# facebookresearch/iris

Measured on AMD Instinct MI355X. Metric: bake_shading throughput (shading samples/s: secondary rays traced and shaded), higher is better.
Workload: dtype f32; 1 GPU; bake_shading train-view sequence (15 views evenly spaced among 32 cameras on a circle, one view per step), 1920x1080, SPP=128 per lobe, lobes=[0, 1, 2, 3, 4, 5, 6] (0=diffuse,1-6=specular), synthetic room seed=1 1000990 triangles, SLF H=256, Philox uniforms; pixels_per_view=2073600

## Files before the change

iris_amd/csrc/iris_bake.h:

```cpp
#pragma once
#include "iris_tile.h"

namespace iris {

struct BakeArgs {
    SceneDev sc; EmitDev em; SlfDev slf;
    const float* pos; const float* nrm; const float* wo;
    const float* u2; const int32_t* pix_id;
    int64_t P; int spp; uint64_t seed; uint32_t stream_id; float rough;
    float* out0; float* out1; int64_t* tri_next;
    int64_t* src_next;
    unsigned long long* stats;
    uint32_t* stack_ovf;
    float4* scratch;
    unsigned int* tile_counter;
    int tile_px;
};

#ifndef IRIS_TILE_RAYS
#define IRIS_TILE_RAYS 5120
#endif
constexpr int kTileRays = IRIS_TILE_RAYS;

__device__ __forceinline__ void reduce_geometry(int spp, int& lpp, int& ppw, int& rounds) {
    if (spp >= 64) { lpp = 64; ppw = 1; rounds = (spp + 63) >> 6; }
    else if ((spp & (spp - 1)) == 0) { lpp = spp; ppw = 64 / spp; rounds = 1; }
    else { lpp = 64; ppw = 1; rounds = 1; }
}

struct RayOut { float r0, g0, b0, r1, g1, b1; };

template <bool SPEC>
__device__ __forceinline__ void sample_dir(const BakeArgs& a, float u0, float u1, f3 n, f3 w, f3 t, f3 b, f3& wi, float& g0, float& g1) {
    g0 = 1.f; g1 = 0.f;
    if (SPEC) {
        wi = specular_sampler(u0, u1, a.rough, w, n, t, b);
        SpecW sw = specular_weights(wi, w, n, a.rough, false);
        g0 = sw.g0; g1 = sw.g1;
    } else {
        wi = diffuse_sampler(u0, u1, n, t, b);
    }
}
template <bool SPEC>
__device__ __forceinline__ void sample_lobe(const BakeArgs& a, int64_t p, int s, f3 n, f3 w, f3 t, f3 b, uint64_t base, f3& wi, float& g0, float& g1) {
    float u0, u1;
    if (a.u2) { const float* up = a.u2 + (p * a.spp + s) * 2; u0 = up[0]; u1 = up[1]; }
    else {
        uint32_t s_lo = (uint32_t)a.seed, s_hi = (uint32_t)(a.seed >> 32);
        asm volatile("" : "+s"(s_lo), "+s"(s_hi));
        philox_u2(((uint64_t)s_hi << 32) | s_lo, base + (uint64_t)s, a.stream_id, u0, u1);
    }
    sample_dir<SPEC>(a, u0, u1, n, w, t, b, wi, g0, g1);
}

template <bool SPEC, bool COUNT, int LAYOUT, int LDS_DEPTH = kStackLds, bool GLOBAL_OVF = false>
__device__ __forceinline__ RayOut trace_shade(const BakeArgs& a, int64_t p, int s, f3 x, f3 wi, float g0, float g1, uint32_t* lds_stack,
                                              TraceStats* ts, uint32_t& n_rays, uint32_t* ovf = nullptr) {
    f3 o = mk3(x.x + kRayEps * wi.x, x.y + kRayEps * wi.y, x.z + kRayEps * wi.z);
    const uint32_t steps0 = COUNT ? ts->nodes + ts->tris : 0;
    Hit h = trace_bvh4<LAYOUT, COUNT, LDS_DEPTH, GLOBAL_OVF>(a.sc, o, wi, lds_stack, ts, ovf);
    if (COUNT) {
        n_rays++;
        uint32_t mine = ts->nodes + ts->tris - steps0, mx = mine;
        for (int m = 1; m < 64; m <<= 1) mx = max(mx, (uint32_t)__shfl_xor((int)mx, m));
        if (first_active_lane()) ts->max_steps64 += (unsigned long long)mx * 64ull;
    }
    f3 pn = mk3(0.f, 0.f, 0.f);
    int64_t tri = -1;
    if (h.slot >= 0) {
        f3 p0, p1, p2;
        hit_vertices(a.sc, h, p0, p1, p2);
        pn = hit_position(h, p0, p1, p2);
        tri = h.id;
    }
    if (a.tri_next) a.tri_next[p * a.spp + s] = tri;
    float epdf; bool vn; int src;
    f3 Le = eval_emitter1(a.em, a.slf, pn, tri, true, 1.0f, 0.0f, epdf, vn, src);
    if (a.src_next) a.src_next[p * a.spp + s] = src;
    RayOut r;
    if (SPEC) { r.r0 = Le.x * g0; r.g0 = Le.y * g0; r.b0 = Le.z * g0; r.r1 = Le.x * g1; r.g1 = Le.y * g1; r.b1 = Le.z * g1; }
    else { r.r0 = Le.x; r.g0 = Le.y; r.b0 = Le.z; r.r1 = r.g1 = r.b1 = 0.f; }
    return r;
}

template <bool SPEC, bool COUNT, int LAYOUT, int LDS_DEPTH = kStackLds, bool GLOBAL_OVF = false>
__device__ __forceinline__ RayOut shade_sample(const BakeArgs& a, int64_t p, int s, f3 x, f3 n, f3 w, f3 t, f3 b, uint64_t base,
                                               uint32_t* lds_stack, TraceStats* ts, uint32_t& n_rays, uint32_t* ovf = nullptr) {
    f3 wi; float g0, g1;
    sample_lobe<SPEC>(a, p, s, n, w, t, b, base, wi, g0, g1);
    return trace_shade<SPEC, COUNT, LAYOUT, LDS_DEPTH, GLOBAL_OVF>(a, p, s, x, wi, g0, g1, lds_stack, ts, n_rays, ovf);
}

template <bool COUNT>
__device__ __forceinline__ void flush_stats(const BakeArgs& a, const TraceStats& ts, uint32_t n_rays) {
    if (COUNT) {
        uint32_t v[8] = {n_rays, ts.nodes, ts.tris, ts.node_iters, ts.leaf_iters, ts.sp_gt8, ts.sp_gt12, ts.sp_gt16};
        for (int k = 0; k < 8; ++k) {
            uint32_t x = v[k];
            for (int m = 1; m < 64; m <<= 1) x += __shfl_xor(x, m);
            if ((threadIdx.x & 63) == 0) atomicAdd(a.stats + k, (unsigned long long)x);
        }
        uint32_t w[2] = {ts.drain_nodes, ts.drain_node_iters};
        for (int k = 0; k < 2; ++k) {
            uint32_t x = w[k];
            for (int m = 1; m < 64; m <<= 1) x += __shfl_xor(x, m);
            if ((threadIdx.x & 63) == 0) atomicAdd(a.stats + 9 + k, (unsigned long long)x);
        }
        uint32_t tp[4] = {ts.top21, ts.top85, ts.top341, ts.top1365};
        for (int k = 0; k < 4; ++k) {
            uint32_t x = tp[k];
            for (int m = 1; m < 64; m <<= 1) x += __shfl_xor(x, m);
            if ((threadIdx.x & 63) == 0) atomicAdd(a.stats + 11 + k, (unsigned long long)x);
        }
        uint32_t sh[5] = {ts.shared_iters, ts.shared_lanes, ts.shared_all_iters, ts.slow_push_iters, ts.shared_path_iters};
        for (int k = 0; k < 5; ++k) {
            uint32_t x = sh[k];
            for (int m = 1; m < 64; m <<= 1) x += __shfl_xor(x, m);
            if ((threadIdx.x & 63) == 0) atomicAdd(a.stats + 15 + k, (unsigned long long)x);
        }
        unsigned long long y = ts.max_steps64;
        for (int m = 1; m < 64; m <<= 1) y += __shfl_xor(y, m);
        if ((threadIdx.x & 63) == 0) atomicAdd(a.stats + 8, y);
    }
}

template <bool SPEC, bool COUNT, int LAYOUT>
__global__ __launch_bounds__(kBlock) void bake_kernel(BakeArgs a) {
    __shared__ uint32_t s_stack[kStackLds * kBlock];
    const int lane = threadIdx.x & 63;
    const int spp = a.spp;
    int lpp, ppw, rounds;
    reduce_geometry(spp, lpp, ppw, rounds);
    const int sub = lane / lpp, sl = lane - sub * lpp;
    const int64_t n_groups = (a.P + ppw - 1) / ppw;
    const int64_t wave0 = ((int64_t)blockIdx.x * kBlock + threadIdx.x) >> 6;
    const int64_t n_waves = ((int64_t)gridDim.x * kBlock) >> 6;
    const float inv_spp = 1.0f / (float)spp;
    TraceStats ts;
    uint32_t n_rays = 0;

    for (int64_t g = wave0; g < n_groups; g += n_waves) {
        const int64_t p = g * ppw + sub;
        const bool pvalid = p < a.P;
        f3 x = mk3(0.f, 0.f, 0.f), n = mk3(0.f, 0.f, 1.f), w = mk3(0.f, 0.f, 1.f), t, b;
        uint64_t base = 0;
        if (pvalid) {
            x = ld3(a.pos + p * 3); n = ld3(a.nrm + p * 3);
            if (SPEC) w = ld3(a.wo + p * 3);
            base = (uint64_t)(a.pix_id ? (int64_t)a.pix_id[p] : p) * (uint64_t)spp;
        }
        normal_space(n, t, b);
        float a0x = 0.f, a0y = 0.f, a0z = 0.f, a1x = 0.f, a1y = 0.f, a1z = 0.f;
        for (int r = 0; r < rounds; ++r) {
            const int s = r * 64 + sl;
            if (pvalid && s < spp) {
                RayOut o = shade_sample<SPEC, COUNT, LAYOUT>(a, p, s, x, n, w, t, b, base, s_stack + threadIdx.x, &ts, n_rays);
                a0x += o.r0; a0y += o.g0; a0z += o.b0;
                if (SPEC) { a1x += o.r1; a1y += o.g1; a1z += o.b1; }
            }
        }
        for (int m = 1; m < lpp; m <<= 1) {
            a0x += __shfl_xor(a0x, m); a0y += __shfl_xor(a0y, m); a0z += __shfl_xor(a0z, m);
            if (SPEC) { a1x += __shfl_xor(a1x, m); a1y += __shfl_xor(a1y, m); a1z += __shfl_xor(a1z, m); }
        }
        if (pvalid && sl == 0) {
            st3(a.out0 + p * 3, mk3(a0x * inv_spp, a0y * inv_spp, a0z * inv_spp));
            if (SPEC) st3(a.out1 + p * 3, mk3(a1x * inv_spp, a1y * inv_spp, a1z * inv_spp));
        }
    }
    flush_stats<COUNT>(a, ts, n_rays);
}

#ifndef IRIS_TILE_WAVES
#define IRIS_TILE_WAVES 7
#endif
#ifndef IRIS_TILE_STACK
#define IRIS_TILE_STACK 12
#endif

template <bool SPEC, bool COUNT, int LAYOUT, int TILE_STACK>
__device__ __forceinline__ void tile_body(const BakeArgs& a, int64_t p0, int np, float4* res, uint16_t* s_sorted, uint32_t* s_stack, int* s_chunk,
                                          uint32_t* ovf, TraceStats& ts, uint32_t& n_rays) {
    const int tid = threadIdx.x, lane = tid & 63, wave = tid >> 6;
    const int spp = a.spp;
    float2* res_g = reinterpret_cast<float2*>(res + kTileRays);
    int lpp, ppw, rounds;
    reduce_geometry(spp, lpp, ppw, rounds);
    const int sub = lane / lpp, sl = lane - sub * lpp;
    const float inv_spp = 1.0f / (float)spp;
    const int nr = np * spp;
    const bool resolve = !a.em.emit_ord && !a.tri_next;

    const uint32_t spp_m = spp > 1 ? (uint32_t)(0x100000000ull / (uint64_t)(uint32_t)spp) + 1u : 0u;
    auto div_spp = [&](int r) -> int { return spp > 1 ? (int)__umulhi((uint32_t)r, spp_m) : r; };

    constexpr int kFrameOff = (kTileRays + 2 * 256 * 4) / 4, kFramePx = (TILE_STACK * kBlock - kFrameOff) / 6;
    float* s_frames = reinterpret_cast<float*>(s_stack) + kFrameOff;
    const bool frames = np <= kFramePx;
    if (frames) {
        for (int pl = tid; pl < np; pl += kBlock) {
            f3 t, b;
            normal_space(ld3(a.nrm + (p0 + pl) * 3), t, b);
            float* f = s_frames + pl * 6;
            f[0] = t.x; f[1] = t.y; f[2] = t.z; f[3] = b.x; f[4] = b.y; f[5] = b.z;
        }
        __syncthreads();
    }

    tile_sort_trace<LAYOUT, COUNT, kTileRays, TILE_STACK, true>(
        a.sc, nr, s_sorted, s_stack, s_chunk, ovf, ts,
        [&](int r) -> uint32_t {
            const int pl = div_spp(r), s = r - pl * spp;
            const int64_t p = p0 + pl;
            const f3 n = ld3(a.nrm + p * 3), w = SPEC ? ld3(a.wo + p * 3) : mk3(0.f, 0.f, 1.f);
            const uint64_t base = (uint64_t)(a.pix_id ? (int64_t)a.pix_id[p] : p) * (uint64_t)spp;
            f3 t, b;
            if (frames) { const float* f = s_frames + pl * 6; t = mk3(f[0], f[1], f[2]); b = mk3(f[3], f[4], f[5]); }
            else normal_space(n, t, b);
            f3 wi; float g0, g1;
            sample_lobe<SPEC>(a, p, s, n, w, t, b, base, wi, g0, g1);
            res[r] = make_float4(wi.x, wi.y, wi.z, 0.f);
            if (SPEC) res_g[r] = make_float2(g1, g0);
            return dir_bin(wi);
        },
        [&](int r, f3& o, f3& d) {
            const int64_t p = p0 + div_spp(r);
            o = ld3(a.pos + p * 3);
            const float4 qa = res[r];
            d = mk3(qa.x, qa.y, qa.z);
        },
        [&](f3& o, f3& d) { o = mk3(o.x + kRayEps * d.x, o.y + kRayEps * d.y, o.z + kRayEps * d.z); },
        [&](int r, const Hit& h) {
            if (resolve) {
                float4 q = make_float4(0.f, 0.f, 0.f, __int_as_float(-2));
                if (h.slot >= 0) {
                    const float4* tr = a.sc.tris + (int64_t)h.slot * 4;
                    const float4 tx = tr[0], ty = tr[1], tz = tr[2];
                    const float ow = tr[3].x;
                    const f3 pn = hit_position(h, mk3(tx.x, ty.x, tz.x), mk3(tx.y, ty.y, tz.y), mk3(tx.z, ty.z, tz.z));
                    q = make_float4(pn.x, pn.y, pn.z, ow);
                }
                res[r] = q;
            } else
            res[r] = make_float4(h.u, h.v, __int_as_float(h.slot), 0.f);
            if (COUNT) n_rays++; }
        );

    const int n_groups = (np + ppw - 1) / ppw;
    IRIS_PHASE_BEGIN();
    for (int g = wave; g < n_groups; g += kBlock / 64) {
        const int pl = g * ppw + sub;
        const bool pvalid = pl < np;
        float a0x = 0.f, a0y = 0.f, a0z = 0.f, a1x = 0.f, a1y = 0.f, a1z = 0.f;
        if (resolve) {
            for (int rr = 0; rr < rounds; rr += 2) {
                const int s0 = rr * 64 + sl, s1 = s0 + 64;
                const bool ok0 = pvalid && s0 < spp, ok1 = pvalid && rr + 1 < rounds && s1 < spp;
                float4 q0 = make_float4(0.f, 0.f, 0.f, __int_as_float(-2)), q1 = q0;
                float2 w0 = make_float2(0.f, 0.f), w1 = w0;
                if (ok0) { q0 = res[pl * spp + s0]; if (SPEC) w0 = res_g[pl * spp + s0]; }
                if (ok1) { q1 = res[pl * spp + s1]; if (SPEC) w1 = res_g[pl * spp + s1]; }
                const int o0 = __float_as_int(q0.w), o1 = __float_as_int(q1.w);
                int j0 = -1, j1 = -1;
                if (o0 == -1) j0 = slf_index(a.slf, mk3(q0.x, q0.y, q0.z));
                if (o1 == -1) j1 = slf_index(a.slf, mk3(q1.x, q1.y, q1.z));
                float4 r0 = make_float4(0.f, 0.f, 0.f, 0.f), r1 = r0;
                if (o0 >= 0 || j0 >= 0) r0 = *(o0 >= 0 ? a.em.radiance + o0 : a.slf.radiance + j0);
                if (o1 >= 0 || j1 >= 0) r1 = *(o1 >= 0 ? a.em.radiance + o1 : a.slf.radiance + j1);
                if (ok0) {
                    const float z = o0 >= 0 ? -0.f : 0.f;
                    const f3 Le = mk3(z + r0.x, z + r0.y, z + r0.z);
                    if (a.src_next) a.src_next[(p0 + pl) * spp + s0] = o0 >= 0 ? -2 - o0 : j0;
                    if (SPEC) { a0x += Le.x * w0.y; a0y += Le.y * w0.y; a0z += Le.z * w0.y; a1x += Le.x * w0.x; a1y += Le.y * w0.x; a1z += Le.z * w0.x; }
                    else { a0x += Le.x; a0y += Le.y; a0z += Le.z; }
                }
                if (ok1) {
                    const float z = o1 >= 0 ? -0.f : 0.f;
                    const f3 Le = mk3(z + r1.x, z + r1.y, z + r1.z);
                    if (a.src_next) a.src_next[(p0 + pl) * spp + s1] = o1 >= 0 ? -2 - o1 : j1;
                    if (SPEC) { a0x += Le.x * w1.y; a0y += Le.y * w1.y; a0z += Le.z * w1.y; a1x += Le.x * w1.x; a1y += Le.y * w1.x; a1z += Le.z * w1.x; }
                    else { a0x += Le.x; a0y += Le.y; a0z += Le.z; }
                }
            }
        } else
        for (int rr = 0; rr < rounds; ++rr) {
            const int s = rr * 64 + sl;
            if (pvalid && s < spp) {
                const float4 qa = res[pl * spp + s];
                Hit h; h.u = qa.x; h.v = qa.y; h.slot = __float_as_int(qa.z); h.t = 0.f; h.id = 0;
                f3 pn = mk3(0.f, 0.f, 0.f);
                int64_t tri = -1;
                int ord_rec = -1;
                if (h.slot >= 0) {
                    const float4* tr = a.sc.tris + (int64_t)h.slot * 4;
                    const float4 tx = tr[0], ty = tr[1], tz = tr[2];
                    if (!a.em.emit_ord) ord_rec = __float_as_int(tr[3].x);
                    pn = hit_position(h, mk3(tx.x, ty.x, tz.x), mk3(tx.y, ty.y, tz.y), mk3(tx.z, ty.z, tz.z));
                    tri = __float_as_int(tx.w);
                }
                if (a.tri_next) a.tri_next[(p0 + pl) * spp + s] = tri;
                float epdf; bool vn; int src;
                const f3 Le = eval_emitter1(a.em, a.slf, pn, tri, true, 1.0f, 0.0f, epdf, vn, src, ord_rec);
                if (a.src_next) a.src_next[(p0 + pl) * spp + s] = src;
                if (SPEC) {
                    const float2 qb = res_g[pl * spp + s];
                    a0x += Le.x * qb.y; a0y += Le.y * qb.y; a0z += Le.z * qb.y;
                    a1x += Le.x * qb.x; a1y += Le.y * qb.x; a1z += Le.z * qb.x;
                } else { a0x += Le.x; a0y += Le.y; a0z += Le.z; }
            }
        }
        for (int m = 1; m < lpp; m <<= 1) {
            a0x += __shfl_xor(a0x, m); a0y += __shfl_xor(a0y, m); a0z += __shfl_xor(a0z, m);
            if (SPEC) { a1x += __shfl_xor(a1x, m); a1y += __shfl_xor(a1y, m); a1z += __shfl_xor(a1z, m); }
        }
        if (pvalid && sl == 0) {
            const int64_t p = p0 + pl;
            st3(a.out0 + p * 3, mk3(a0x * inv_spp, a0y * inv_spp, a0z * inv_spp));
            if (SPEC) st3(a.out1 + p * 3, mk3(a1x * inv_spp, a1y * inv_spp, a1z * inv_spp));
        }
    }
    IRIS_PHASE_MARK(3);
}

constexpr int kTileChunk = 64;
__device__ __forceinline__ long long claim_tile(unsigned int* counters, long long n_tiles) {
    constexpr int kChunk = kTileChunk;
    const long long n_chunks = (n_tiles + kChunk - 1) / kChunk;
    for (int k = 0; k < 8; ++k) {
        const int x = ((int)blockIdx.x + k) & 7;
        const long long per = (n_chunks + 7 - x) / 8;
        for (;;) {
            const unsigned int c = atomicAdd(counters + x, 1u);
            const long long ch = (long long)(c / kChunk);
            if (ch >= per) break;
            const long long t = (ch * 8 + x) * kChunk + (c % kChunk);
            if (t < n_tiles) return t;
        }
    }
    return n_tiles;
}

template <bool SPEC, bool COUNT, int LAYOUT>
__global__ __launch_bounds__(kBlock, COUNT ? 4 : IRIS_TILE_WAVES) void bake_tile_kernel(BakeArgs a) {
    constexpr int kTileStack = IRIS_TILE_STACK;
    __shared__ uint16_t s_sorted[kTileRays];
    __shared__ uint32_t s_stack[kTileStack * kBlock];
    __shared__ int s_tile, s_chunk;
    static_assert(kTileStack * kBlock * 4 >= kTileRays + 2 * 256 * 4, "stack region too small to alias the sort keys");
    const int tid = threadIdx.x;
    constexpr int NC = SPEC ? 2 : 1;
    float4* res = a.scratch + (size_t)blockIdx.x * kTileRays * NC;
    uint32_t* ovf = a.stack_ovf + (size_t)blockIdx.x * (kStackCapacity - kTileStack) * kBlock;
    const int64_t n_tiles = (a.P + a.tile_px - 1) / a.tile_px;
    TraceStats ts;
    uint32_t n_rays = 0;
    for (;;) {
        __syncthreads();
        if (tid == 0) { s_tile = (int)claim_tile(a.tile_counter, n_tiles); s_chunk = 0; }
        (s_stack + kTileRays / 4)[tid] = 0;
        __syncthreads();
        const int64_t tile = s_tile;
        if (tile >= n_tiles) break;
        const int64_t p0 = (int64_t)tile * a.tile_px;
        tile_body<SPEC, COUNT, LAYOUT, kTileStack>(a, p0, (int)min((int64_t)a.tile_px, a.P - p0), res, s_sorted, s_stack, &s_chunk, ovf, ts, n_rays);
    }
    flush_stats<COUNT>(a, ts, n_rays);
}

constexpr int kMaxLobes = 8;
struct ViewLobe { float rough; int spp; uint32_t stream_id; int spec; int tile_px; int tiles_per_span; float* out0; float* out1; };
struct ViewArgs {
    BakeArgs base;
    int n_lobes;
    int span_px;
    long long n_tiles;
    ViewLobe lobe[kMaxLobes];
};

template <int LAYOUT>
__global__ __launch_bounds__(kBlock, IRIS_TILE_WAVES) void bake_view_kernel(ViewArgs v) {
    constexpr int kTileStack = IRIS_TILE_STACK;
    __shared__ uint16_t s_sorted[kTileRays];
    __shared__ uint32_t s_stack[kTileStack * kBlock];
    __shared__ int s_tile, s_chunk;
    static_assert(kTileStack * kBlock * 4 >= kTileRays + 2 * 256 * 4, "stack region too small to alias the sort keys");
    const int tid = threadIdx.x;
    float4* res = v.base.scratch + (size_t)blockIdx.x * kTileRays * 2;
    uint32_t* ovf = v.base.stack_ovf + (size_t)blockIdx.x * (kStackCapacity - kTileStack) * kBlock;
    for (;;) {
        __syncthreads();
        if (tid == 0) { s_tile = (int)claim_tile(v.base.tile_counter, v.n_tiles); s_chunk = 0; }
        (s_stack + kTileRays / 4)[tid] = 0;
        __syncthreads();
        const long long vt = s_tile;
        if (vt >= v.n_tiles) break;
        const long long g = vt / kTileChunk, q = g >> 3;
        const int j = (int)(vt % kTileChunk), l = (int)(q % v.n_lobes);
        const int64_t span0 = ((q / v.n_lobes) * 8 + (g & 7)) * (int64_t)v.span_px;
        const int64_t p0 = span0 + (int64_t)j * v.lobe[l].tile_px;
        if (j >= v.lobe[l].tiles_per_span || p0 >= v.base.P) continue;
        const int np = (int)min((int64_t)v.lobe[l].tile_px, min(v.base.P, span0 + v.span_px) - p0);
        BakeArgs a = v.base;
        a.spp = v.lobe[l].spp; a.rough = v.lobe[l].rough; a.stream_id = v.lobe[l].stream_id; a.tile_px = v.lobe[l].tile_px;
        a.out0 = v.lobe[l].out0; a.out1 = v.lobe[l].out1; a.u2 = nullptr; a.tri_next = nullptr; a.src_next = nullptr;
        TraceStats ts; uint32_t n_rays = 0;
        if (v.lobe[l].spec) tile_body<true, false, LAYOUT, kTileStack>(a, p0, np, res, s_sorted, s_stack, &s_chunk, ovf, ts, n_rays);
        else tile_body<false, false, LAYOUT, kTileStack>(a, p0, np, res, s_sorted, s_stack, &s_chunk, ovf, ts, n_rays);
    }
}

}
```

iris_amd/csrc/iris_tile.h:

```cpp
#pragma once
#include "iris_trace.h"

namespace iris {

#ifndef IRIS_PRIO_A
#define IRIS_PRIO_A 0
#endif
#ifndef IRIS_PRIO_C
#define IRIS_PRIO_C 3
#endif
#ifndef IRIS_PRIO_D
#define IRIS_PRIO_D 0
#endif

__device__ __forceinline__ uint32_t dir_bin(f3 d) {
    const float ax = fabsf(d.x), ay = fabsf(d.y), az = fabsf(d.z);
    const float inv = __builtin_amdgcn_rcpf(ax + ay + az + 1e-30f);
    const float a = ax * inv, b = ay * inv;
    const float v = b * __builtin_amdgcn_rcpf(1.f - a + 1e-30f);
    const int iu = min(7, (int)(a * 8.f)), iv0 = min(3, (int)(v * 4.f));
    const int iv = (iu & 1) ? 3 - iv0 : iv0;
    const uint32_t oct = (d.x < 0.f ? 1u : 0u) | (d.y < 0.f ? 2u : 0u) | (d.z < 0.f ? 4u : 0u);
    return (oct << 5) | ((uint32_t)iu << 2) | (uint32_t)iv;
}

#ifdef IRIS_PHASE_TIMING
__device__ unsigned long long g_phase_cycles[8];
#define IRIS_PHASE_BEGIN() unsigned long long t_phase_ = clock64()
#define IRIS_PHASE_MARK(k) do { if (threadIdx.x == 0) { const unsigned long long t_ = clock64(); atomicAdd(&g_phase_cycles[k], t_ - t_phase_); t_phase_ = t_; } } while (0)
#else
#define IRIS_PHASE_BEGIN()
#define IRIS_PHASE_MARK(k)
#endif

template <int LAYOUT, bool COUNT, int CAP, int TILE_STACK, bool GLOBAL_OVF, class PhaseA, class FetchRay, class Prepare, class Retire>
__device__ __forceinline__ void tile_sort_trace(const SceneDev& sc, int nr, uint16_t* s_sorted, uint32_t* s_stack, int* s_chunk, uint32_t* ovf,
                                                TraceStats& ts, PhaseA phase_a, FetchRay fetch_ray, Prepare prepare, Retire retire) {
    static_assert(TILE_STACK * kBlock * 4 >= CAP + 2 * 256 * 4, "stack region too small to alias the sort keys");
    uint8_t* s_keys = reinterpret_cast<uint8_t*>(s_stack);
    uint32_t* s_hist = s_stack + CAP / 4;
    uint32_t* s_cur = s_hist + 256;
    const int tid = threadIdx.x, lane = tid & 63, wave = tid >> 6;
    IRIS_PHASE_BEGIN();
    __builtin_amdgcn_s_setprio(IRIS_PRIO_A);
    for (int r = tid; r < nr; r += kBlock) {
        const uint32_t key = phase_a(r);
        s_keys[r] = (uint8_t)key;
        atomicAdd(&s_hist[key], 1u);
    }
    __syncthreads();
    IRIS_PHASE_MARK(0);
    if (wave == 0) {
        uint32_t c0 = s_hist[lane * 4], c1 = s_hist[lane * 4 + 1], c2 = s_hist[lane * 4 + 2], c3 = s_hist[lane * 4 + 3];
        uint32_t tot = c0 + c1 + c2 + c3, inc = tot;
        for (int m = 1; m < 64; m <<= 1) { uint32_t v = __shfl_up(inc, m); if (lane >= m) inc += v; }
        uint32_t ex = inc - tot;
        s_cur[lane * 4] = ex; s_cur[lane * 4 + 1] = ex + c0; s_cur[lane * 4 + 2] = ex + c0 + c1; s_cur[lane * 4 + 3] = ex + c0 + c1 + c2;
    }
    __syncthreads();
    for (int r = tid; r < nr; r += kBlock) {
        const uint32_t pos = atomicAdd(&s_cur[s_keys[r]], 1u);
        s_sorted[pos] = (uint16_t)r;
    }
    __syncthreads();
    IRIS_PHASE_MARK(1);
    {
        int my_r = 0;
        auto fetch = [&](f3& o, f3& d) -> bool {
            const unsigned long long m = __ballot(1);
            int base = 0;
            if (lane == __ffsll((long long)m) - 1) base = atomicAdd(s_chunk, __popcll(m));
            base = __builtin_amdgcn_readfirstlane(base);
            const int i = base + (int)__builtin_amdgcn_mbcnt_hi((uint32_t)(m >> 32), __builtin_amdgcn_mbcnt_lo((uint32_t)m, 0u));
            if (i >= nr) return false;
            my_r = s_sorted[i];
            fetch_ray(my_r, o, d);
            return true;
        };
        auto ret = [&](const Hit& h) { retire(my_r, h); };
        __builtin_amdgcn_s_setprio(IRIS_PRIO_C);
        uint32_t tid_c = threadIdx.x;
        asm volatile("" : "+v"(tid_c));
        SceneDev sc_c = sc;
        asm volatile("" : "+s"(sc_c.nodes), "+s"(sc_c.tris), "+s"(sc_c.oct_stride));
        trace_stream<LAYOUT, COUNT, TILE_STACK, GLOBAL_OVF>(sc_c, s_stack + tid_c, tid_c, ovf, &ts, fetch, prepare, ret);
        __builtin_amdgcn_s_setprio(IRIS_PRIO_D);
        IRIS_PHASE_MARK(4);
    }
    __syncthreads();
    IRIS_PHASE_MARK(2);
}

}
```

Before: 9229 Mrays/s.

## Outline sampling and shading phases into noinline functions reading kernel args directly

Splits the per-tile body into separate noinline functions for sample generation/binning (phase A) and shading/accumulation (phase D). Each reloads its arguments from the kernel-argument segment, with wave-uniform parameters and global address-space pointers, and the traversal loop stays inlined. The aim is to stop register pressure from the sampling and shading code from inflating the traversal's register allocation, and to merge the spec and diffuse paths so only one traversal instance is compiled per kernel. The trade-off is call overhead, possible spills at call boundaries, and reliance on the implicit-argument layout of the kernel arguments.

```diff
diff --git a/iris_amd/csrc/iris_bake.h b/iris_amd/csrc/iris_bake.h
--- a/iris_amd/csrc/iris_bake.h
+++ b/iris_amd/csrc/iris_bake.h
@@ -178,22 +178,67 @@
 #define IRIS_TILE_STACK 12
 #endif
 
-template <bool SPEC, bool COUNT, int LAYOUT, int TILE_STACK>
-__device__ __forceinline__ void tile_body(const BakeArgs& a, int64_t p0, int np, float4* res, uint16_t* s_sorted, uint32_t* s_stack, int* s_chunk,
-                                          uint32_t* ovf, TraceStats& ts, uint32_t& n_rays) {
-    const int tid = threadIdx.x, lane = tid & 63, wave = tid >> 6;
+typedef __attribute__((address_space(4))) const char cst_char;
+template <class ARGS> __device__ __forceinline__ cst_char* kernel_args() { return (cst_char*)__builtin_amdgcn_implicitarg_ptr() - ((sizeof(ARGS) + 7) & ~(size_t)7); }
+template <class T> __device__ __forceinline__ T* as_global(T* p) { return (T*)(__attribute__((address_space(1))) T*)p; }
+__device__ __forceinline__ void globalize(BakeArgs& a) {
+    a.sc.tris = as_global(a.sc.tris); a.em.emit_ord = as_global(a.em.emit_ord); a.em.radiance = as_global(a.em.radiance);
+    a.slf.inds = as_global(a.slf.inds); a.slf.radiance = as_global(a.slf.radiance);
+    a.nrm = as_global(a.nrm); a.wo = as_global(a.wo); a.u2 = as_global(a.u2); a.pix_id = as_global(a.pix_id);
+    a.out0 = as_global(a.out0); a.out1 = as_global(a.out1); a.tri_next = as_global(a.tri_next); a.src_next = as_global(a.src_next); a.scratch = as_global(a.scratch);
+}
+struct ViewLobe { float rough; int spp; uint32_t stream_id; int spec; int tile_px; int tiles_per_span; float* out0; float* out1; };
+__device__ __forceinline__ void set_lobe(BakeArgs& a, const ViewLobe& L) {
+    a.spp = L.spp; a.rough = L.rough; a.stream_id = L.stream_id; a.tile_px = L.tile_px;
+    a.out0 = L.out0; a.out1 = L.out1; a.u2 = nullptr; a.tri_next = nullptr; a.src_next = nullptr;
+}
+constexpr int kMaxLobes = 8;
+struct ViewArgs {
+    BakeArgs base;
+    int n_lobes;
+    int span_px;
+    long long n_tiles;
+    ViewLobe lobe[kMaxLobes];
+};
+struct TileLaunch {
+    typedef BakeArgs Args;
+    template <bool SPEC> static constexpr int kSlab = SPEC ? 2 : 1;
+    __device__ static __forceinline__ BakeArgs args(cst_char* k, int) {
+        BakeArgs a;
+        __builtin_memcpy(&a, k, sizeof(BakeArgs));
+        globalize(a);
+        return a;
+    }
+};
+struct ViewLaunch {
+    typedef ViewArgs Args;
+    template <bool SPEC> static constexpr int kSlab = 2;
+    __device__ static __forceinline__ BakeArgs args(cst_char* k, int l) {
+        BakeArgs a; ViewLobe L;
+        __builtin_memcpy(&a, k + offsetof(ViewArgs, base), sizeof(BakeArgs));
+        __builtin_memcpy(&L, k + offsetof(ViewArgs, lobe) + (size_t)l * sizeof(ViewLobe), sizeof(ViewLobe));
+        set_lobe(a, L);
+        globalize(a);
+        return a;
+    }
+};
+#define IRIS_TILE_PHASE __device__ __noinline__
+__device__ __forceinline__ int64_t uniform64(int64_t x) {
+    return (int64_t)(((uint64_t)(uint32_t)__builtin_amdgcn_readfirstlane((int)((uint64_t)x >> 32)) << 32) | (uint32_t)__builtin_amdgcn_readfirstlane((int)x));
+}
+
+
+template <bool SPEC, int TILE_STACK, class LAUNCH>
+IRIS_TILE_PHASE void tile_phase_a(int l, int64_t p0, int np, lds_u32* lds) {
+    l = __builtin_amdgcn_readfirstlane(l); np = __builtin_amdgcn_readfirstlane(np); p0 = uniform64(p0);
+    const BakeArgs a = LAUNCH::args(kernel_args<typename LAUNCH::Args>(), l);
+    uint32_t* s_stack = (uint32_t*)lds;
+    float4* res = a.scratch + (size_t)blockIdx.x * kTileRays * LAUNCH::template kSlab<SPEC>;
+    float2* res_g = reinterpret_cast<float2*>(res + kTileRays);
+    const int tid = threadIdx.x;
     const int spp = a.spp;
-    float2* res_g = reinterpret_cast<float2*>(res + kTileRays);
-    int lpp, ppw, rounds;
-    reduce_geometry(spp, lpp, ppw, rounds);
-    const int sub = lane / lpp, sl = lane - sub * lpp;
-    const float inv_spp = 1.0f / (float)spp;
-    const int nr = np * spp;
-    const bool resolve = !a.em.emit_ord && !a.tri_next;
-
     const uint32_t spp_m = spp > 1 ? (uint32_t)(0x100000000ull / (uint64_t)(uint32_t)spp) + 1u : 0u;
     auto div_spp = [&](int r) -> int { return spp > 1 ? (int)__umulhi((uint32_t)r, spp_m) : r; };
-
     constexpr int kFrameOff = (kTileRays + 2 * 256 * 4) / 4, kFramePx = (TILE_STACK * kBlock - kFrameOff) / 6;
     float* s_frames = reinterpret_cast<float*>(s_stack) + kFrameOff;
     const bool frames = np <= kFramePx;
@@ -207,8 +252,7 @@
         __syncthreads();
     }
 
-    tile_sort_trace<LAYOUT, COUNT, kTileRays, TILE_STACK, true>(
-        a.sc, nr, s_sorted, s_stack, s_chunk, ovf, ts,
+    tile_bin<kTileRays>(np * spp, s_stack,
         [&](int r) -> uint32_t {
             const int pl = div_spp(r), s = r - pl * spp;
             const int64_t p = p0 + pl;
@@ -222,30 +266,22 @@
             res[r] = make_float4(wi.x, wi.y, wi.z, 0.f);
             if (SPEC) res_g[r] = make_float2(g1, g0);
             return dir_bin(wi);
-        },
-        [&](int r, f3& o, f3& d) {
-            const int64_t p = p0 + div_spp(r);
-            o = ld3(a.pos + p * 3);
-            const float4 qa = res[r];
-            d = mk3(qa.x, qa.y, qa.z);
-        },
-        [&](f3& o, f3& d) { o = mk3(o.x + kRayEps * d.x, o.y + kRayEps * d.y, o.z + kRayEps * d.z); },
-        [&](int r, const Hit& h) {
-            if (resolve) {
-                float4 q = make_float4(0.f, 0.f, 0.f, __int_as_float(-2));
-                if (h.slot >= 0) {
-                    const float4* tr = a.sc.tris + (int64_t)h.slot * 4;
-                    const float4 tx = tr[0], ty = tr[1], tz = tr[2];
-                    const float ow = tr[3].x;
-                    const f3 pn = hit_position(h, mk3(tx.x, ty.x, tz.x), mk3(tx.y, ty.y, tz.y), mk3(tx.z, ty.z, tz.z));
-                    q = make_float4(pn.x, pn.y, pn.z, ow);
-                }
-                res[r] = q;
-            } else
-            res[r] = make_float4(h.u, h.v, __int_as_float(h.slot), 0.f);
-            if (COUNT) n_rays++; }
-        );
-
+        });
+}
+
+template <bool SPEC, class LAUNCH>
+IRIS_TILE_PHASE void tile_phase_d(int l, int64_t p0, int np) {
+    l = __builtin_amdgcn_readfirstlane(l); np = __builtin_amdgcn_readfirstlane(np); p0 = uniform64(p0);
+    const BakeArgs a = LAUNCH::args(kernel_args<typename LAUNCH::Args>(), l);
+    float4* res = a.scratch + (size_t)blockIdx.x * kTileRays * LAUNCH::template kSlab<SPEC>;
+    float2* res_g = reinterpret_cast<float2*>(res + kTileRays);
+    const int tid = threadIdx.x, lane = tid & 63, wave = tid >> 6;
+    const int spp = a.spp;
+    int lpp, ppw, rounds;
+    reduce_geometry(spp, lpp, ppw, rounds);
+    const int sub = lane / lpp, sl = lane - sub * lpp;
+    const float inv_spp = 1.0f / (float)spp;
+    const bool resolve = !a.em.emit_ord && !a.tri_next;
     const int n_groups = (np + ppw - 1) / ppw;
     IRIS_PHASE_BEGIN();
     for (int g = wave; g < n_groups; g += kBlock / 64) {
@@ -322,6 +358,58 @@
     IRIS_PHASE_MARK(3);
 }
 
+template <bool SPEC, int TILE_STACK> struct TileLobe {
+    __device__ __forceinline__ void phase_a(int64_t p0, int np, uint32_t* s_stack) const { tile_phase_a<SPEC, TILE_STACK, TileLaunch>(0, p0, np, (lds_u32*)s_stack); }
+    __device__ __forceinline__ void phase_d(int64_t p0, int np) const { tile_phase_d<SPEC, TileLaunch>(0, p0, np); }
+};
+template <int TILE_STACK> struct ViewTileLobe {
+    int l; bool spec;
+    __device__ __forceinline__ void phase_a(int64_t p0, int np, uint32_t* s_stack) const {
+        if (spec) tile_phase_a<true, TILE_STACK, ViewLaunch>(l, p0, np, (lds_u32*)s_stack); else tile_phase_a<false, TILE_STACK, ViewLaunch>(l, p0, np, (lds_u32*)s_stack);
+    }
+    __device__ __forceinline__ void phase_d(int64_t p0, int np) const {
+        if (spec) tile_phase_d<true, ViewLaunch>(l, p0, np); else tile_phase_d<false, ViewLaunch>(l, p0, np);
+    }
+};
+
+template <bool COUNT, int LAYOUT, int TILE_STACK, class LOBE>
+__device__ __forceinline__ void tile_body(const BakeArgs& a, LOBE lobe, int64_t p0, int np, float4* res, uint16_t* s_sorted, uint32_t* s_stack, int* s_chunk,
+                                          uint32_t* ovf, TraceStats& ts, uint32_t& n_rays) {
+    const int spp = a.spp;
+    const int nr = np * spp;
+    const bool resolve = !a.em.emit_ord && !a.tri_next;
+    const uint32_t spp_m = spp > 1 ? (uint32_t)(0x100000000ull / (uint64_t)(uint32_t)spp) + 1u : 0u;
+    auto div_spp = [&](int r) -> int { return spp > 1 ? (int)__umulhi((uint32_t)r, spp_m) : r; };
+
+    lobe.phase_a(p0, np, s_stack);
+    tile_trace_sorted<LAYOUT, COUNT, kTileRays, TILE_STACK, true>(
+        a.sc, nr, s_sorted, s_stack, s_chunk, ovf, ts,
+        [&](int r, f3& o, f3& d) {
+            const int64_t p = p0 + div_spp(r);
+            o = ld3(a.pos + p * 3);
+            const float4 qa = res[r];
+            d = mk3(qa.x, qa.y, qa.z);
+        },
+        [&](f3& o, f3& d) { o = mk3(o.x + kRayEps * d.x, o.y + kRayEps * d.y, o.z + kRayEps * d.z); },
+        [&](int r, const Hit& h) {
+            if (resolve) {
+                float4 q = make_float4(0.f, 0.f, 0.f, __int_as_float(-2));
+                if (h.slot >= 0) {
+                    const float4* tr = a.sc.tris + (int64_t)h.slot * 4;
+                    const float4 tx = tr[0], ty = tr[1], tz = tr[2];
+                    const float ow = tr[3].x;
+                    const f3 pn = hit_position(h, mk3(tx.x, ty.x, tz.x), mk3(tx.y, ty.y, tz.y), mk3(tx.z, ty.z, tz.z));
+                    q = make_float4(pn.x, pn.y, pn.z, ow);
+                }
+                res[r] = q;
+            } else
+            res[r] = make_float4(h.u, h.v, __int_as_float(h.slot), 0.f);
+            if (COUNT) n_rays++; }
+        );
+
+    lobe.phase_d(p0, np);
+}
+
 constexpr int kTileChunk = 64;
 __device__ __forceinline__ long long claim_tile(unsigned int* counters, long long n_tiles) {
     constexpr int kChunk = kTileChunk;
@@ -362,20 +450,11 @@
         const int64_t tile = s_tile;
         if (tile >= n_tiles) break;
         const int64_t p0 = (int64_t)tile * a.tile_px;
-        tile_body<SPEC, COUNT, LAYOUT, kTileStack>(a, p0, (int)min((int64_t)a.tile_px, a.P - p0), res, s_sorted, s_stack, &s_chunk, ovf, ts, n_rays);
+        tile_body<COUNT, LAYOUT, kTileStack>(a, TileLobe<SPEC, kTileStack>(), p0, (int)min((int64_t)a.tile_px, a.P - p0), res, s_sorted, s_stack, &s_chunk, ovf, ts, n_rays);
     }
     flush_stats<COUNT>(a, ts, n_rays);
 }
 
-constexpr int kMaxLobes = 8;
-struct ViewLobe { float rough; int spp; uint32_t stream_id; int spec; int tile_px; int tiles_per_span; float* out0; float* out1; };
-struct ViewArgs {
-    BakeArgs base;
-    int n_lobes;
-    int span_px;
-    long long n_tiles;
-    ViewLobe lobe[kMaxLobes];
-};
 
 template <int LAYOUT>
 __global__ __launch_bounds__(kBlock, IRIS_TILE_WAVES) void bake_view_kernel(ViewArgs v) {
@@ -401,12 +480,10 @@
         if (j >= v.lobe[l].tiles_per_span || p0 >= v.base.P) continue;
         const int np = (int)min((int64_t)v.lobe[l].tile_px, min(v.base.P, span0 + v.span_px) - p0);
         BakeArgs a = v.base;
-        a.spp = v.lobe[l].spp; a.rough = v.lobe[l].rough; a.stream_id = v.lobe[l].stream_id; a.tile_px = v.lobe[l].tile_px;
-        a.out0 = v.lobe[l].out0; a.out1 = v.lobe[l].out1; a.u2 = nullptr; a.tri_next = nullptr; a.src_next = nullptr;
+        set_lobe(a, v.lobe[l]);
         TraceStats ts; uint32_t n_rays = 0;
-        if (v.lobe[l].spec) tile_body<true, false, LAYOUT, kTileStack>(a, p0, np, res, s_sorted, s_stack, &s_chunk, ovf, ts, n_rays);
-        else tile_body<false, false, LAYOUT, kTileStack>(a, p0, np, res, s_sorted, s_stack, &s_chunk, ovf, ts, n_rays);
-    }
-}
-
-}
+        tile_body<false, LAYOUT, kTileStack>(a, ViewTileLobe<kTileStack>{l, v.lobe[l].spec != 0}, p0, np, res, s_sorted, s_stack, &s_chunk, ovf, ts, n_rays);
+    }
+}
+
+}
diff --git a/iris_amd/csrc/iris_tile.h b/iris_amd/csrc/iris_tile.h
--- a/iris_amd/csrc/iris_tile.h
+++ b/iris_amd/csrc/iris_tile.h
@@ -33,14 +33,12 @@
 #define IRIS_PHASE_MARK(k)
 #endif
 
-template <int LAYOUT, bool COUNT, int CAP, int TILE_STACK, bool GLOBAL_OVF, class PhaseA, class FetchRay, class Prepare, class Retire>
-__device__ __forceinline__ void tile_sort_trace(const SceneDev& sc, int nr, uint16_t* s_sorted, uint32_t* s_stack, int* s_chunk, uint32_t* ovf,
-                                                TraceStats& ts, PhaseA phase_a, FetchRay fetch_ray, Prepare prepare, Retire retire) {
-    static_assert(TILE_STACK * kBlock * 4 >= CAP + 2 * 256 * 4, "stack region too small to alias the sort keys");
+
+template <int CAP, class PhaseA>
+__device__ __forceinline__ void tile_bin(int nr, uint32_t* s_stack, PhaseA phase_a) {
     uint8_t* s_keys = reinterpret_cast<uint8_t*>(s_stack);
     uint32_t* s_hist = s_stack + CAP / 4;
-    uint32_t* s_cur = s_hist + 256;
-    const int tid = threadIdx.x, lane = tid & 63, wave = tid >> 6;
+    const int tid = threadIdx.x;
     IRIS_PHASE_BEGIN();
     __builtin_amdgcn_s_setprio(IRIS_PRIO_A);
     for (int r = tid; r < nr; r += kBlock) {
@@ -50,6 +48,17 @@
     }
     __syncthreads();
     IRIS_PHASE_MARK(0);
+}
+
+template <int LAYOUT, bool COUNT, int CAP, int TILE_STACK, bool GLOBAL_OVF, class FetchRay, class Prepare, class Retire>
+__device__ __forceinline__ void tile_trace_sorted(const SceneDev& sc, int nr, uint16_t* s_sorted, uint32_t* s_stack, int* s_chunk, uint32_t* ovf,
+                                                  TraceStats& ts, FetchRay fetch_ray, Prepare prepare, Retire retire) {
+    static_assert(TILE_STACK * kBlock * 4 >= CAP + 2 * 256 * 4, "stack region too small to alias the sort keys");
+    uint8_t* s_keys = reinterpret_cast<uint8_t*>(s_stack);
+    uint32_t* s_hist = s_stack + CAP / 4;
+    uint32_t* s_cur = s_hist + 256;
+    const int tid = threadIdx.x, lane = tid & 63, wave = tid >> 6;
+    IRIS_PHASE_BEGIN();
     if (wave == 0) {
         uint32_t c0 = s_hist[lane * 4], c1 = s_hist[lane * 4 + 1], c2 = s_hist[lane * 4 + 2], c3 = s_hist[lane * 4 + 3];
         uint32_t tot = c0 + c1 + c2 + c3, inc = tot;
@@ -91,4 +100,11 @@
     IRIS_PHASE_MARK(2);
 }
 
+template <int LAYOUT, bool COUNT, int CAP, int TILE_STACK, bool GLOBAL_OVF, class PhaseA, class FetchRay, class Prepare, class Retire>
+__device__ __forceinline__ void tile_sort_trace(const SceneDev& sc, int nr, uint16_t* s_sorted, uint32_t* s_stack, int* s_chunk, uint32_t* ovf,
+                                                TraceStats& ts, PhaseA phase_a, FetchRay fetch_ray, Prepare prepare, Retire retire) {
+    tile_bin<CAP>(nr, s_stack, phase_a);
+    tile_trace_sorted<LAYOUT, COUNT, CAP, TILE_STACK, GLOBAL_OVF>(sc, nr, s_sorted, s_stack, s_chunk, ovf, ts, fetch_ray, prepare, retire);
 }
+
+}
```

Result: no change. 9148 Mrays/s (-0.9%).

## Skip tracing specular samples with zero lobe weight in tile sort

Applied to the files above, without the earlier changes.

Specular samples whose lobe weights are both zero are marked dead during the sort phase. They are left out of the direction histogram and the sorted list, and the shared chunk counter starts past them, so no BVH traversal runs for them. Their result slot is preset to a miss/zero record so the later shading pass gives a zero contribution. The gain depends on how often lobe sampling gives zero weight (e.g. below-horizon directions). The cost is a per-thread bitmask that limits tile capacity and extra branching in phase A.

```diff
diff --git a/iris_amd/csrc/iris_bake.h b/iris_amd/csrc/iris_bake.h
--- a/iris_amd/csrc/iris_bake.h
+++ b/iris_amd/csrc/iris_bake.h
@@ -83,11 +83,14 @@
     return r;
 }
 
+__device__ __forceinline__ bool dead_samples_skippable(const BakeArgs& a) { return !a.tri_next && !a.src_next; }
+
 template <bool SPEC, bool COUNT, int LAYOUT, int LDS_DEPTH = kStackLds, bool GLOBAL_OVF = false>
 __device__ __forceinline__ RayOut shade_sample(const BakeArgs& a, int64_t p, int s, f3 x, f3 n, f3 w, f3 t, f3 b, uint64_t base,
                                                uint32_t* lds_stack, TraceStats* ts, uint32_t& n_rays, uint32_t* ovf = nullptr) {
     f3 wi; float g0, g1;
     sample_lobe<SPEC>(a, p, s, n, w, t, b, base, wi, g0, g1);
+    if (SPEC && !COUNT && dead_samples_skippable(a) && g0 == 0.f && g1 == 0.f) return RayOut{0.f, 0.f, 0.f, 0.f, 0.f, 0.f};
     return trace_shade<SPEC, COUNT, LAYOUT, LDS_DEPTH, GLOBAL_OVF>(a, p, s, x, wi, g0, g1, lds_stack, ts, n_rays, ovf);
 }
 
@@ -190,6 +193,7 @@
     const float inv_spp = 1.0f / (float)spp;
     const int nr = np * spp;
     const bool resolve = !a.em.emit_ord && !a.tri_next;
+    const bool skip_dead = dead_samples_skippable(a);
 
     const uint32_t spp_m = spp > 1 ? (uint32_t)(0x100000000ull / (uint64_t)(uint32_t)spp) + 1u : 0u;
     auto div_spp = [&](int r) -> int { return spp > 1 ? (int)__umulhi((uint32_t)r, spp_m) : r; };
@@ -207,7 +211,7 @@
         __syncthreads();
     }
 
-    tile_sort_trace<LAYOUT, COUNT, kTileRays, TILE_STACK, true>(
+    tile_sort_trace<LAYOUT, COUNT, kTileRays, TILE_STACK, true, SPEC && !COUNT>(
         a.sc, nr, s_sorted, s_stack, s_chunk, ovf, ts,
         [&](int r) -> uint32_t {
             const int pl = div_spp(r), s = r - pl * spp;
@@ -219,9 +223,10 @@
             else normal_space(n, t, b);
             f3 wi; float g0, g1;
             sample_lobe<SPEC>(a, p, s, n, w, t, b, base, wi, g0, g1);
-            res[r] = make_float4(wi.x, wi.y, wi.z, 0.f);
             if (SPEC) res_g[r] = make_float2(g1, g0);
-            return dir_bin(wi);
+            const bool dead = SPEC && !COUNT && skip_dead && g0 == 0.f && g1 == 0.f;
+            res[r] = dead ? make_float4(0.f, 0.f, __int_as_float(resolve ? 0 : -1), __int_as_float(resolve ? -2 : 0)) : make_float4(wi.x, wi.y, wi.z, 0.f);
+            return dead ? kDeadRay : dir_bin(wi);
         },
         [&](int r, f3& o, f3& d) {
             const int64_t p = p0 + div_spp(r);
diff --git a/iris_amd/csrc/iris_tile.h b/iris_amd/csrc/iris_tile.h
--- a/iris_amd/csrc/iris_tile.h
+++ b/iris_amd/csrc/iris_tile.h
@@ -33,16 +33,27 @@
 #define IRIS_PHASE_MARK(k)
 #endif
 
-template <int LAYOUT, bool COUNT, int CAP, int TILE_STACK, bool GLOBAL_OVF, class PhaseA, class FetchRay, class Prepare, class Retire>
+constexpr uint32_t kDeadRay = 256u;
+template <int LAYOUT, bool COUNT, int CAP, int TILE_STACK, bool GLOBAL_OVF, bool SKIP_DEAD = false, class PhaseA, class FetchRay, class Prepare, class Retire>
 __device__ __forceinline__ void tile_sort_trace(const SceneDev& sc, int nr, uint16_t* s_sorted, uint32_t* s_stack, int* s_chunk, uint32_t* ovf,
                                                 TraceStats& ts, PhaseA phase_a, FetchRay fetch_ray, Prepare prepare, Retire retire) {
     static_assert(TILE_STACK * kBlock * 4 >= CAP + 2 * 256 * 4, "stack region too small to alias the sort keys");
+    static_assert(!SKIP_DEAD || CAP <= 32 * kBlock, "one bit per ray of a thread");
     uint8_t* s_keys = reinterpret_cast<uint8_t*>(s_stack);
     uint32_t* s_hist = s_stack + CAP / 4;
     uint32_t* s_cur = s_hist + 256;
     const int tid = threadIdx.x, lane = tid & 63, wave = tid >> 6;
     IRIS_PHASE_BEGIN();
     __builtin_amdgcn_s_setprio(IRIS_PRIO_A);
+    uint32_t dead = 0;
+    if (SKIP_DEAD) {
+        uint32_t bit = 1u;
+        for (int r = tid; r < nr; r += kBlock, bit <<= 1) {
+            const uint32_t key = phase_a(r);
+            if (key == kDeadRay) dead |= bit;
+            else { s_keys[r] = (uint8_t)key; atomicAdd(&s_hist[key], 1u); }
+        }
+    } else
     for (int r = tid; r < nr; r += kBlock) {
         const uint32_t key = phase_a(r);
         s_keys[r] = (uint8_t)key;
@@ -55,9 +66,21 @@
         uint32_t tot = c0 + c1 + c2 + c3, inc = tot;
         for (int m = 1; m < 64; m <<= 1) { uint32_t v = __shfl_up(inc, m); if (lane >= m) inc += v; }
         uint32_t ex = inc - tot;
+        if (SKIP_DEAD) {
+            const uint32_t first = (uint32_t)nr - (uint32_t)__builtin_amdgcn_readlane((int)inc, 63);
+            ex += first;
+            if (lane == 0) *s_chunk = (int)first;
+        }
         s_cur[lane * 4] = ex; s_cur[lane * 4 + 1] = ex + c0; s_cur[lane * 4 + 2] = ex + c0 + c1; s_cur[lane * 4 + 3] = ex + c0 + c1 + c2;
     }
     __syncthreads();
+    if (SKIP_DEAD) {
+        for (int r = tid; r < nr; r += kBlock, dead >>= 1) {
+            if (dead & 1u) continue;
+            const uint32_t pos = atomicAdd(&s_cur[s_keys[r]], 1u);
+            s_sorted[pos] = (uint16_t)r;
+        }
+    } else
     for (int r = tid; r < nr; r += kBlock) {
         const uint32_t pos = atomicAdd(&s_cur[s_keys[r]], 1u);
         s_sorted[pos] = (uint16_t)r;
```

New measurement: 9235 Mrays/s before, 10510 Mrays/s after, median of 6. +13.8%, better.
